# uzh-rpg/ess

Hardware: AMD Instinct MI355X
Metric: UDA train-step throughput (voxel grids/s = N*B*T/step_time) (higher is better)
Workload: dtype f16 forward / bf16 backward

## Files before the change

### ess_amd/csrc/conv_wgrad.hip

```cpp
#include "conv_wgrad_common.h"
#include <stdlib.h>

namespace {


__device__ __forceinline__ float load_virtual(const WgradArgs& a, int n, int c, int gy, int gx) {
  const bool first = c < a.C0;
  const int mode = first ? a.mode0 : a.mode1;
  const int sh = mode != ESS_SRC_DIRECT ? 1 : 0;
  const int Hp = a.Hin >> sh, Wp = a.Win >> sh;
  const float* sp = first ? a.src0 : a.src1;
  const int cc = first ? c : c - a.C0, Cs = first ? a.C0 : a.C1;
  const bool ok = gy >= 0 && gy < a.Hin && gx >= 0 && gx < a.Win && !(mode == ESS_SRC_ZERO_UP2 && ((gy | gx) & 1));
  const int cy = min(max(gy, 0), a.Hin - 1) >> sh, cx = min(max(gx, 0), a.Win - 1) >> sh;
  const float t = sp[(((size_t)n * Cs + cc) * Hp + cy) * Wp + cx];
  return ok ? t : 0.f;
}

__device__ __forceinline__ void load8_virtual(const WgradArgs& a, int n, int c, int gy, int gx, bool valid, float (&f)[8]) {
  const bool first = c < a.C0;
  const int mode = first ? a.mode0 : a.mode1;
  const float* sp = first ? a.src0 : a.src1;
  const int cc = first ? c : c - a.C0, Cs = first ? a.C0 : a.C1;
  const bool rowok = valid && gy >= 0 && gy < a.Hin;
// ... 686 lines not shown
  if (a.ws_b && tid < Cout) a.ws_b[(size_t)blockIdx.x * Cout + tid] = (redb[0][tid] + redb[1][tid]) + (redb[2][tid] + redb[3][tid]);
}

struct TapMap { int mapped; signed char m[12]; };
template <int E, int NT, int THREADS>
__global__ __launch_bounds__(THREADS) void wgrad_reduce_kernel(const float* ws, const float* ws_b, float* dw, float* db, int nsplit, int T,
                                                           int CC, int Cout, int nblk_w, int accumulate, const TapMap tm) {
  constexpr int G = THREADS / E, PITCH = E * NT + 1, U = NT == 1 ? 8 : 4;
  __shared__ float part[G * PITCH];
  int blk = blockIdx.x, t0 = blockIdx.y * NT, nt = min(NT, T - t0);
  if (blk >= nblk_w) {
    if (blockIdx.y) return;
    blk -= nblk_w; ws = ws_b; dw = db; T = 1; CC = Cout; nt = 1;
  }
  const bool mapped = tm.mapped && T == 9;
  const int el = threadIdx.x % E, g = threadIdx.x / E;
  const int e = blk * E + el;
  float acc[NT];
#pragma unroll
  for (int u = 0; u < NT; ++u) acc[u] = 0.f;
  if (e < CC) {
    int k = g;
    for (; k + (U - 1) * G < nsplit; k += U * G) {
      float v[U][NT];
#pragma unroll
      for (int j = 0; j < U; ++j) {
        const float* src = ws + ((size_t)(k + j * G) * T + t0) * CC + e;
#pragma unroll
        for (int u = 0; u < NT; ++u) v[j][u] = u < nt ? src[(size_t)u * CC] : 0.f;
      }
#pragma unroll
      for (int u = 0; u < NT; ++u) {
        float t = 0.f;
#pragma unroll
        for (int j = 0; j < U; j += 2) t += v[j][u] + v[j + 1][u];
        acc[u] += t;
      }
    }
    for (; k < nsplit; k += G) {
      const float* src = ws + ((size_t)k * T + t0) * CC + e;
#pragma unroll
      for (int u = 0; u < NT; ++u)
        if (u < nt) acc[u] += src[(size_t)u * CC];
    }
  }
#pragma unroll
  for (int u = 0; u < NT; ++u) part[g * PITCH + el * NT + u] = acc[u];
  __syncthreads();
  for (int idx = threadIdx.x; idx < E * NT; idx += THREADS) {
    const int l = idx / NT, u = idx - l * NT;
    if (u < nt && blk * E + l < CC) {
      float t = 0.f;
#pragma unroll
      for (int w = 0; w < G; ++w) t += part[w * PITCH + idx];
      const int td = mapped ? tm.m[t0 + u] : t0 + u;
      if (td < 0) continue;
      float* dst = dw + (size_t)(blk * E + l) * T + td;
      *dst = accumulate ? *dst + t : t;
    }
  }
}

enum WRoute {
  W_F32_TILE,
  W_TAPS7,
  W_BF16_K3,
  W_BF16_K3_FAST,
  W_BF16_K1,
  W_C8_K3,
  W_C8_K1,
  W_SMALL1X1,
  W_SMALL1X1_MFMA,
  W_SMALL1X1_C8X
};
inline bool tile128(WRoute r) { return r == W_BF16_K3 || r == W_BF16_K3_FAST || r == W_BF16_K1 || r == W_C8_K3 || r == W_C8_K1; }

struct WPlan {
  EssConvDesc d;
  WRoute route;
  bool phases;
  WgradBArgs args;
  unsigned grid;
  int lds_bytes;
  size_t ws_bytes;
};

inline bool k3s1p1(const EssConvDesc* d) { return d->ksize == 3 && d->stride == 1 && d->pad == 1; }

inline bool s2_phases(const EssConvDesc* d) {
  return d->fmt0 == ESS_FMT_BF16_C8 && d->fmt_out == ESS_FMT_BF16_C8 && d->ksize == 3 && d->stride == 2 && d->pad == 1 && d->C1 == 0 &&
         d->mode0 == ESS_SRC_DIRECT && d->H_in == 2 * d->H_out && d->W_in == 2 * d->W_out;
}
inline EssConvDesc s2_phase_desc(const EssConvDesc* d) {
  EssConvDesc p = *d;
  p.stride = 1; p.H_in = d->H_out; p.W_in = d->W_out; p.mode1 = ESS_SRC_DIRECT;
  return p;
}
inline TapMap s2_phase_taps(int p, int q) {
  TapMap tm{};
  tm.mapped = 1;
  for (int t = 0; t < 9; ++t) {
    const int kyp = t / 3, kxp = t % 3;
    const int ky = p == 0 ? (kyp == 1 ? 1 : -1) : (kyp == 0 ? 0 : kyp == 1 ? 2 : -1);
    const int kx = q == 0 ? (kxp == 1 ? 1 : -1) : (kxp == 0 ? 0 : kxp == 1 ? 2 : -1);
    tm.m[t] = (signed char)((ky < 0 || kx < 0) ? -1 : ky * 3 + kx);
  }
  return tm;
}

int wvalidate(const EssConvDesc* d) {
  ESS_CHECK_ARG(d != nullptr, "wgrad: null descriptor");
  ESS_CHECK_ARG(d->epilogue == ESS_EPI_LINEAR && d->out_split == 0, "wgrad: only plain convolutions have a weight gradient here");
  ESS_CHECK_ARG(d->mode0 >= ESS_SRC_DIRECT && d->mode0 <= ESS_SRC_ZERO_UP2 && d->mode1 >= ESS_SRC_DIRECT && d->mode1 <= ESS_SRC_ZERO_UP2,
                "wgrad: source modes DIRECT / NEAREST_UP2 / ZERO_UP2 only (the space-to-depth form exists for the frozen encoder's forward)");
  const int cin = d->C0 + d->C1;
  const bool taps = cin == 1 && d->ksize == 7;
  ESS_CHECK_ARG(taps || d->ksize == 1 || d->ksize == 3, "wgrad: k=%d with C_in=%d unsupported", d->ksize, cin);
  ESS_CHECK_ARG(d->stride == 1 || d->stride == 2, "wgrad: stride %d unsupported", d->stride);
  const bool xc8 = d->fmt0 == ESS_FMT_BF16_C8, dc8 = d->fmt_out == ESS_FMT_BF16_C8;
  ESS_CHECK_ARG(d->compute == ESS_COMPUTE_FP32 || d->compute == ESS_COMPUTE_BF16 || d->compute == ESS_COMPUTE_BF16X3, "wgrad: bad compute type");
  if (xc8 || dc8) {
    ESS_CHECK_ARG(d->compute == ESS_COMPUTE_BF16, "wgrad: BF16_C8 tensors need bf16 compute");
    ESS_CHECK_ARG(d->C1 == 0 || d->fmt1 == d->fmt0, "wgrad: both sources of a concat must use the same format");
    ESS_CHECK_ARG(d->C1 == 0 || (d->C0 % 8) == 0, "wgrad: the first BF16_C8 source of a concat must have a multiple of 8 channels");
    if (xc8 && dc8)
      ESS_CHECK_ARG(k3s1p1(d) || (d->ksize == 1 && d->pad == 0 && d->mode0 == ESS_SRC_DIRECT && d->C1 == 0) || s2_phases(d),
                    "wgrad(BF16_C8): 3x3 / stride 1 / pad 1, 3x3 / stride 2 / pad 1 on even extents (one direct source) and 1x1 / pad 0 convolutions only");
    else if (xc8)
      ESS_CHECK_ARG(d->ksize == 1 && d->stride == 1 && d->pad == 0 && d->C1 == 0 && d->mode0 == ESS_SRC_DIRECT && d->C_out <= 32 && cin <= 32,
                    "wgrad(BF16_C8 X, fp32 dY): the 1x1 head only (C_in, C_out <= 32)");
    else
      ESS_CHECK_ARG(taps, "wgrad(fp32 X, BF16_C8 dY): the 7x7 single-channel stem only");
  }
  return ESS_OK;
}

WRoute wroute(const EssConvDesc* d) {
  const int cin = d->C0 + d->C1, KS = d->ksize;
  const bool xc8 = d->fmt0 == ESS_FMT_BF16_C8, dc8 = d->fmt_out == ESS_FMT_BF16_C8;
  if (xc8 && dc8) return KS == 3 ? W_C8_K3 : W_C8_K1;
  if (xc8) return W_SMALL1X1_C8X;
  const bool k1s1p0 = KS == 1 && d->stride == 1 && d->pad == 0;
  if (k1s1p0 && d->C1 == 0 && d->mode0 == ESS_SRC_DIRECT && d->C_out <= 16 && cin <= 64)
    return cin <= 32 && ((d->H_out * d->W_out) % 64) == 0 ? W_SMALL1X1_MFMA : W_SMALL1X1;
  const bool rows8 = (d->W_in % 8) == 0 && (d->W_out % 8) == 0 && d->mode0 != ESS_SRC_ZERO_UP2 && d->mode1 != ESS_SRC_ZERO_UP2;
  if (d->compute == ESS_COMPUTE_BF16 && k3s1p1(d)) return rows8 ? W_BF16_K3_FAST : W_BF16_K3;
  if (d->compute == ESS_COMPUTE_BF16 && k1s1p0 && rows8) return W_BF16_K1;
  if (cin == 1 && KS == 7) return W_TAPS7;
  return W_F32_TILE;
}

WPlan wplan(const EssConvDesc* desc) {
  WPlan w{};
  w.d = *desc;
  if (desc->compute == ESS_COMPUTE_BF16X3) {
    w.args.split = k3s1p1(desc);
    w.d.compute = w.args.split ? ESS_COMPUTE_BF16 : ESS_COMPUTE_FP32;
  }
  w.phases = s2_phases(&w.d);
  if (w.phases) w.d = s2_phase_desc(&w.d);
  const EssConvDesc* d = &w.d;
  w.route = wroute(d);
  WgradArgs& a = w.args.w;
  a.N = d->N; a.Hin = d->H_in; a.Win = d->W_in; a.C0 = d->C0; a.C1 = d->C1; a.mode0 = d->mode0; a.mode1 = d->mode1;
  a.Cout = d->C_out; a.Hout = d->H_out; a.Wout = d->W_out;
  a.pad = (w.route == W_BF16_K1 || w.route == W_C8_K1) ? 1 : d->pad;
  a.dy_c8 = d->fmt_out == ESS_FMT_BF16_C8;
  a.ps = w.phases;
  const int cin = d->C0 + d->C1, KS = d->ksize, S = d->stride;
  const bool wide = tile128(w.route);
  const int npx = wide ? 128 : 64;
  double best = 1e300;
  for (int twl = 5; twl >= (wide ? 4 : 3); --twl) {
    const int tw = 1 << twl, th = npx >> twl;
    const double c = (double)ceil_div(d->W_out, tw) * tw * ceil_div(d->H_out, th) * th + 1e-3 * (5 - twl);
    if (c < best) { best = c; a.twl = twl; }
  }
  if (w.route == W_C8_K3) a.twl = 4;
  const int tw = 1 << a.twl, th = npx >> a.twl;
  a.tiles_x = ceil_div(d->W_out, tw); a.tiles_y = ceil_div(d->H_out, th);
  a.ntiles = d->N * a.tiles_x * a.tiles_y;
  a.IH = (th - 1) * S + KS; a.IW = (tw - 1) * S + KS;
  a.plx = (a.IH * a.IW) | 1;
  a.ci_tiles = w.route == W_TAPS7 ? 1 : ceil_div(cin, 64);
  a.npairs = ceil_div(d->C_out, 64) * a.ci_tiles;
  const size_t slab_floats = (size_t)KS * KS * d->C_out * cin + d->C_out;
  int ns = wide ? ceil_div(256, a.npairs) : ceil_div(2048, a.npairs);
  if (ns > a.ntiles) ns = a.ntiles;
  const size_t cap = ((size_t)64 << 20) / (slab_floats * 4);
  if ((size_t)ns > cap) ns = (int)(cap ? cap : 1);
  if (ns < 1) ns = 1;
  if (w.route == W_SMALL1X1 || w.route == W_SMALL1X1_C8X) {
    const int chunks = d->N * ceil_div(d->H_out * d->W_out, 128);
    ns = chunks < 1024 ? chunks : 1024;
  } else if (w.route == W_SMALL1X1_MFMA) {
    const int groups = d->N * (d->H_out * d->W_out / 64);
    ns = groups < 4 * 512 ? ceil_div(groups, 4) : 512;
  }
  a.nsplit = ns;
  w.grid = (unsigned)(a.npairs * ns);
  w.ws_bytes = (size_t)ns * slab_floats * 4;
  w.lds_bytes = (64 * 65 + (w.route == W_TAPS7 ? a.IH * a.IW : 64 * a.plx)) * 4;
  if (wide) {
    w.args.rv = tw / 8 + 2;
    w.args.pyv = (th * tw / 8) | 1;
    w.args.pxv = ((th + 2) * w.args.rv) | 1;
    w.lds_bytes = 64 * (w.args.pyv + w.args.pxv) * 16 * (w.route == W_BF16_K3 ? 1 : 2);
  }
  return w;
}

struct WgradSet { const void* x0; const void* x1; const void* dy; };

WgradBArgs wfill(const WPlan& w, const WgradSet& s, void* workspace, bool bias, int ph) {
  WgradBArgs b = w.args;
  WgradArgs& a = b.w;
  a.src0 = (const float*)s.x0; a.src1 = a.C1 ? (const float*)s.x1 : nullptr; a.dy = (const float*)s.dy;
  a.ws = (float*)workspace;
  a.ws_b = bias ? a.ws + (size_t)a.nsplit * w.d.ksize * w.d.ksize * a.Cout * (a.C0 + a.C1) : nullptr;
  a.pp = ph >> 1; a.pq = ph & 1;
  return b;
}

template <typename K, typename... A>
int wgo(K kernel, dim3 grid, int lds_bytes, hipStream_t st, const A&... args) {
  const int rc = wgrad_raise_lds(kernel, lds_bytes);
  if (rc) return rc;
  hipLaunchKernelGGL(kernel, grid, dim3(256), lds_bytes, st, args...);
  return ESS_OK;
}

int wlaunch(const WPlan& w, WRoute route, const WgradBArgs& b, hipStream_t st) {
  const EssConvDesc& d = w.d;
  const dim3 grid(w.grid);
  const int px = d.H_out * d.W_out, nsplit = b.w.nsplit;
  int rc = ESS_OK;
  switch (route) {
    case W_F32_TILE: {
      const auto kernel = d.ksize == 3 ? (d.stride == 1 ? wgrad_f32_kernel<3, 1> : wgrad_f32_kernel<3, 2>)
                                       : (d.stride == 1 ? wgrad_f32_kernel<1, 1> : wgrad_f32_kernel<1, 2>);
      rc = wgo(kernel, grid, w.lds_bytes, st, b.w);
      break;
    }
    case W_TAPS7: rc = wgo(wgrad_taps_kernel<7, 2>, grid, w.lds_bytes, st, b.w); break;
    case W_BF16_K3: rc = wgo(wgrad_bf16_k3s1_kernel, grid, w.lds_bytes, st, b); break;
    case W_BF16_K3_FAST: rc = wgo(wgrad_bf16_k3s1_fast_kernel<9>, grid, w.lds_bytes, st, b); break;
    case W_BF16_K1: rc = wgo(wgrad_bf16_k3s1_fast_kernel<1>, grid, w.lds_bytes, st, b); break;
    case W_C8_K3: rc = wgrad_c8_k3_launch(b, grid, st); break;
    case W_C8_K1: rc = wgrad_c8_k1_launch(b, d.stride, w.lds_bytes, grid, st); break;
    case W_SMALL1X1: rc = wgo(wgrad_small1x1_kernel, dim3(nsplit), 0, st, b.w, ceil_div(px, 128), d.N * ceil_div(px, 128)); break;
    case W_SMALL1X1_MFMA: rc = wgo(wgrad_small1x1_mfma_kernel, dim3(nsplit), 0, st, b.w, px / 64, d.N * (px / 64)); break;
    case W_SMALL1X1_C8X: rc = wgrad_small1x1_c8_launch(b.w, nsplit, st); break;
  }
  return rc ? rc : ess_launch_status("conv2d_wgrad");
}

int wreduce(const WPlan& w, const WgradArgs& a, float* dw, float* db, int accumulate, const TapMap& tm, hipStream_t st) {
  const int T = w.d.ksize * w.d.ksize, CC = w.d.C_out * (w.d.C0 + w.d.C1);
  const int nblk_w = ceil_div(CC, 64), nblk_b = a.ws_b ? ceil_div(w.d.C_out, 64) : 0;
  if (T == 9 && CC >= 32768)
    hipLaunchKernelGGL((wgrad_reduce_kernel<64, 9, 256>), dim3((unsigned)(nblk_w + nblk_b)), dim3(256), 0, st, a.ws, a.ws_b, dw, db, a.nsplit, T,
                       CC, w.d.C_out, nblk_w, accumulate, tm);
  else
    hipLaunchKernelGGL((wgrad_reduce_kernel<64, 1, 1024>), dim3((unsigned)(nblk_w + nblk_b), (unsigned)T), dim3(1024), 0, st, a.ws, a.ws_b, dw, db,
                       a.nsplit, T, CC, w.d.C_out, nblk_w, accumulate, tm);
  return ess_launch_status("conv2d_wgrad_reduce");
}

bool env_on(const char* name) {
  const char* e = getenv(name);
  return !(e && e[0] == '0');
}

bool split_via_c8(const EssConvDesc* d) {
  static const bool on = env_on("ESS_X3_WGRAD_C8");
  return on && d->compute == ESS_COMPUTE_BF16X3 && k3s1p1(d) && (d->C1 == 0 || (d->C0 % 8) == 0) && d->mode0 != ESS_SRC_ZERO_UP2 &&
         d->mode1 != ESS_SRC_ZERO_UP2 && (d->C1 == 0 || d->mode1 == ESS_SRC_DIRECT);
}
EssConvDesc c8_desc(const EssConvDesc* d) {
  EssConvDesc c = *d;
  c.compute = ESS_COMPUTE_BF16;
  c.fmt0 = c.fmt1 = c.fmt_out = ESS_FMT_BF16_C8;
  return c;
}
struct SplitCopy { int C, H, W; size_t bytes; };
struct SplitLayout { size_t slabs, total; SplitCopy t[3]; };
SplitLayout split_layout(const EssConvDesc* d) {
  const EssConvDesc dc = c8_desc(d);
  const int s0 = d->mode0 != ESS_SRC_DIRECT ? 1 : 0, s1 = d->mode1 != ESS_SRC_DIRECT ? 1 : 0;
  SplitLayout s{(wplan(&dc).ws_bytes + 255) & ~(size_t)255, 0,
                {{d->C0, d->H_in >> s0, d->W_in >> s0, 0}, {d->C1, d->H_in >> s1, d->W_in >> s1, 0}, {d->C_out, d->H_out, d->W_out, 0}}};
  s.total = s.slabs;
  for (SplitCopy& t : s.t) {
    t.bytes = (((size_t)d->N * ((t.C + 7) / 8) * t.H * t.W * 16) + 255) & ~(size_t)255;
    s.total += 2 * t.bytes;
  }
  return s;
}

int wgrad_split_via_c8(const EssConvDesc* d, const WgradSet& s, float* dw, float* db, int accumulate, void* workspace, size_t workspace_bytes,
                       hipStream_t st);

int wgrad_run(const EssConvDesc* d, int n_sets, const WgradSet* sets, int bias_mask, float* dw, float* db, int accumulate, void* workspace,
              size_t workspace_bytes, hipStream_t st) {
  int rc = wvalidate(d);
  if (rc) return rc;
  ESS_CHECK_ARG(dw && workspace, "wgrad: null pointer");
  uintptr_t bits = 0;
  for (int q = 0; q < n_sets; ++q) {
    ESS_CHECK_ARG(sets[q].x0 && sets[q].dy, "wgrad: null pointer");
    ESS_CHECK_ARG(d->C1 == 0 || sets[q].x1, "wgrad: second source missing");
    bits |= (uintptr_t)sets[q].x0 | (uintptr_t)sets[q].dy | (d->C1 ? (uintptr_t)sets[q].x1 : 0);
  }
  if (split_via_c8(d)) {
    for (int q = 0; q < n_sets; ++q)
      if ((rc = wgrad_split_via_c8(d, sets[q], dw, ((bias_mask >> q) & 1) ? db : nullptr, q ? 1 : accumulate, workspace, workspace_bytes, st))) return rc;
    return ESS_OK;
  }
  const WPlan w = wplan(d);
  ESS_CHECK_ARG(workspace_bytes >= w.ws_bytes, "wgrad: workspace too small");
  ESS_CHECK_ARG(w.lds_bytes <= 160 * 1024, "wgrad: LDS tile %d B too large", w.lds_bytes);
  if (w.d.fmt0 == ESS_FMT_BF16_C8 || w.d.fmt_out == ESS_FMT_BF16_C8)
    ESS_CHECK_ARG((bits & 15) == 0, "wgrad: BF16_C8 tensors must be 16-byte aligned");
  if (w.route == W_TAPS7) {
    ESS_CHECK_ARG(w.d.stride == 2, "wgrad: 7x7 stem variant is stride 2 only");
    ESS_CHECK_ARG(!db, "wgrad: the stem variant has no bias gradient");
  }
  const bool one_launch = n_sets > 1 && w.route == W_C8_K3 && !w.phases;
  for (int q = 0; q < (one_launch ? 1 : n_sets); ++q) {
    const bool misaligned = (((uintptr_t)sets[q].x0 | (uintptr_t)sets[q].dy) & 15) != 0;
    const WRoute route = (w.route == W_SMALL1X1_MFMA && misaligned) ? W_SMALL1X1 : w.route;
    for (int ph = 0; ph < (w.phases ? 4 : 1); ++ph) {
      const bool bias = db && ph == 0 && (one_launch || ((bias_mask >> q) & 1));
      WgradBArgs b = wfill(w, sets[q], workspace, bias, ph);
      if (one_launch) {
        b.npass = n_sets; b.bias_mask = bias_mask;
        for (int i = 0; i < n_sets; ++i) { b.p_dy[i] = sets[i].dy; b.p_x0[i] = sets[i].x0; b.p_x1[i] = d->C1 ? sets[i].x1 : nullptr; }
      }
      if ((rc = wlaunch(w, route, b, st))) return rc;
      if ((rc = wreduce(w, b.w, dw, db, (q || accumulate) ? 1 : 0, w.phases ? s2_phase_taps(ph >> 1, ph & 1) : TapMap{}, st))) return rc;
    }
  }
  return ESS_OK;
}

int wgrad_split_via_c8(const EssConvDesc* d, const WgradSet& s, float* dw, float* db, int accumulate, void* workspace,
                              size_t workspace_bytes, hipStream_t st) {
  int rc;
// ... 46 lines not shown
```

### ess_amd/csrc/conv_wgrad_c8.hip

```cpp
#include "conv_wgrad_common.h"
#include <stdlib.h>
#include <type_traits>

namespace {

struct Quad { u32x4w v[4]; };

__device__ __forceinline__ void quad_transpose(const Quad& q, uint2 (&out)[8]) {
#pragma unroll
  for (int d = 0; d < 4; ++d) {
    out[2 * d].x = __builtin_amdgcn_perm(q.v[1][d], q.v[0][d], 0x05040100u);
    out[2 * d].y = __builtin_amdgcn_perm(q.v[3][d], q.v[2][d], 0x05040100u);
    out[2 * d + 1].x = __builtin_amdgcn_perm(q.v[1][d], q.v[0][d], 0x07060302u);
    out[2 * d + 1].y = __builtin_amdgcn_perm(q.v[3][d], q.v[2][d], 0x07060302u);
  }
}

template <int OFF>
__device__ __forceinline__ void lds_read128(u32x4w& d, unsigned addr) {
  asm volatile("ds_read_b128 %0, %1 offset:%2" : "=v"(d) : "v"(addr), "n"(OFF));
}

template <int TAPS, int TWL>
__global__ __launch_bounds__(256) void wgrad_c8_kernel(const WgradBArgs b, int sx_abl) {
// ... 150 lines not shown
    auto mma = [&](const Frag& f) {
      if (abl & 1) return;
      const bf16x8w af = __builtin_bit_cast(bf16x8w, f.a);
      if (want_b) {
#pragma unroll
        for (int j = 0; j < 8; ++j) bsum += (float)af[j];
      }
      if constexpr (TAPS == 1) {
        acc[0] = __builtin_amdgcn_mfma_f32_32x32x16_bf16(af, __builtin_bit_cast(bf16x8w, f.v[1][1]), acc[0], 0, 0, 0);
      } else {
#pragma unroll
        for (int ky = 0; ky < 3; ++ky) {
          acc[ky * 3 + 0] = __builtin_amdgcn_mfma_f32_32x32x16_bf16(af, __builtin_bit_cast(bf16x8w, shift_left1(f.v[ky][0], f.v[ky][1])),
                                                                    acc[ky * 3 + 0], 0, 0, 0);
          acc[ky * 3 + 1] = __builtin_amdgcn_mfma_f32_32x32x16_bf16(af, __builtin_bit_cast(bf16x8w, f.v[ky][1]), acc[ky * 3 + 1], 0, 0, 0);
          acc[ky * 3 + 2] = __builtin_amdgcn_mfma_f32_32x32x16_bf16(af, __builtin_bit_cast(bf16x8w, shift_right1(f.v[ky][1], f.v[ky][2])),
                                                                    acc[ky * 3 + 2], 0, 0, 0);
        }
      }
    };
    Frag f0, f1;
    ESS_RD(f0, 0)
    ESS_RD(f1, 1) ESS_WT(f0, NR) mma(f0);
    if (more) issue(tile + nsplit);
    ESS_RD(f0, 2) ESS_WT(f1, NR) mma(f1);
    ESS_RD(f1, 3) ESS_WT(f0, NR) mma(f0);
    ESS_RD(f0, 4) ESS_WT(f1, NR) mma(f1);
    if (more) commit_d(st ^ 1);
    ESS_RD(f1, 5) ESS_WT(f0, NR) mma(f0);
    if (more) commit_x(0, st ^ 1);
    ESS_RD(f0, 6) ESS_WT(f1, NR) mma(f1);
    if (more) commit_x(1, st ^ 1);
    ESS_RD(f1, 7) ESS_WT(f0, NR) mma(f0);
    if (more) commit_x(2, st ^ 1);
    ESS_WT(f1, 0) mma(f1);
#undef ESS_RD
#undef ESS_WT
#undef ESS_ROFF
    __syncthreads();
  }
  const int ci = cit * 64 + ib * 32 + p;
  if (abl & 8) return;
#pragma unroll
  for (int t = 0; t < TAPS; ++t)
#pragma unroll
    for (int r = 0; r < 16; ++r) {
      const int co = cot * 64 + cb * 32 + (r & 3) + 8 * (r >> 2) + 4 * half;
      if (co < a.Cout && ci < Cin) a.ws[(((size_t)split * TAPS + t) * a.Cout + co) * Cin + ci] = acc[t][r];
    }
  if (want_b) {
    bsum += __shfl_xor(bsum, 32, 64);
    const int co = cot * 64 + cb * 32 + p;
    if (half == 0 && co < a.Cout) a.ws_b[(size_t)split * a.Cout + co] = bsum;
  }
}

template <int OFF>
__device__ __forceinline__ void lds_read_tr(uint2& d, unsigned addr) {
  asm volatile("ds_read_b64_tr_b16 %0, %1 offset:%2" : "=v"(d) : "v"(addr), "n"(OFF));
}
template <int I, int N, class F>
__device__ __forceinline__ void static_for(F&& f) {
  if constexpr (I < N) {
    f(std::integral_constant<int, I>{});
    static_for<I + 1, N>(f);
  }
}
#define ESS_LDS_PTR(off_) ((__attribute__((address_space(3))) void*)(size_t)(off_))

struct DmaGeom {
  static constexpr int TWL = 4, TW = 16, TH = 8, RW = TW + 2, IH = TH + 2, XPX = IH * RW;
  static constexpr int XP = (XPX + 63) / 64, XTAIL = XPX - (XP - 1) * 64;
  static constexpr int DPL = 2 * 1024 + 64, XPL = XPX * 16;
  static_assert(XPL % 256 == 64, "X plane pitch");
  static constexpr int XREG = 8 * DPL, STAGE = 8 * (DPL + XPL);
};

#ifdef ESS_WG_TRACE
__device__ unsigned long long g_wg_trace[1024 * 8 * 40];
#define ESS_TR(i_) do { if (lane == 0 && blockIdx.x < 1024) g_wg_trace[(blockIdx.x * 8 + wave) * 40 + (i_)] = __builtin_readcyclecounter(); } while (0)
#else
#define ESS_TR(i_) do { } while (0)
#endif
template <int NST>
__global__ __launch_bounds__(512) void wgrad_c8_ws_kernel(const WgradBArgs b) {
  using G = DmaGeom;
  constexpr int PER_WAVE = 2 * (2 + G::XP);
  constexpr int AHEAD = 2;
  static_assert(NST == AHEAD + 2, "stages: tile k - 1 (last two units), k, k + 1 (landing), k + 2 (being issued)");
  extern __shared__ __attribute__((aligned(16))) unsigned char smem_dma[];
  const WgradArgs& a = b.w;
  const int tid = threadIdx.x, lane = tid & 63, wave = __builtin_amdgcn_readfirstlane(tid >> 6), half = lane >> 5, p = lane & 31;
  const bool loader = wave >= 4;
  const int w4 = wave & 3;
  const int logical = xcd_remap(blockIdx.x, gridDim.x);
  const int pair = logical % a.npairs, split = logical / a.npairs, nsplit = a.nsplit;
  const int cot = pair / a.ci_tiles, cit = pair - cot * a.ci_tiles;
  const int Cin = a.C0 + a.C1;
  const unsigned lds0 = (unsigned)(size_t)smem_dma;
  const int ntt = b.npass > 1 ? b.npass * a.ntiles : a.ntiles;
  int ntl = 0;
  if (split < ntt) ntl = (ntt - 1 - split) / nsplit + 1;

  ESS_TR(0);
  if (loader) {
    const int sh0 = a.mode0 != ESS_SRC_DIRECT ? 1 : 0, sh1 = a.mode1 != ESS_SRC_DIRECT ? 1 : 0;
    const bool z0 = a.mode0 == ESS_SRC_ZERO_UP2, z1 = a.mode1 == ESS_SRC_ZERO_UP2;
    const int nbo = (a.Cout + 7) >> 3, nb0 = (a.C0 + 7) >> 3, nb1 = (a.C1 + 7) >> 3;
    const unsigned HWo16 = (unsigned)a.Hout * a.Wout * 16u;
    const int W0 = (a.Win << a.ps) >> sh0, W1 = a.Win >> sh1;
    const unsigned HW0_16 = (unsigned)((a.Hin << a.ps) >> sh0) * W0 * 16u, HW1_16 = (unsigned)(a.Hin >> sh1) * W1 * 16u;
    int d_r[2], d_c[2], x_r[G::XP], x_c[G::XP];
#pragma unroll
    for (int q = 0; q < 2; ++q) { const int pi = q * 64 + lane; d_r[q] = pi >> G::TWL; d_c[q] = pi & (G::TW - 1); }
#pragma unroll
    for (int q = 0; q < G::XP; ++q) { const int pi = q * 64 + lane; x_r[q] = pi / G::RW; x_c[q] = pi % G::RW; }
    unsigned dpl_off[2], xpl_off[2];
    bool xpl_first[2];
#pragma unroll
    for (int j = 0; j < 2; ++j) {
      const int pl = 2 * w4 + j;
      const int ob = cot * 8 + pl;
      dpl_off[j] = ob < nbo ? (unsigned)ob * HWo16 : OOBW;
      const int c0 = (cit * 8 + pl) * 8;
      const bool first = c0 < a.C0 || a.C1 == 0;
      const int bi = (first ? c0 : c0 - a.C0) >> 3;
      xpl_first[j] = first;
      xpl_off[j] = (c0 < Cin && bi < (first ? nb0 : nb1)) ? (unsigned)bi * (first ? HW0_16 : HW1_16) : OOBW;
    }
    const int tpi = a.tiles_x * a.tiles_y;
    auto issue = [&](int tile, int st) {
      const char* p_dy = (const char*)a.dy;
      const char* p_x0 = (const char*)a.src0;
      const char* p_x1 = (const char*)a.src1;
      if (b.npass > 1) {
        const int pass = tile / a.ntiles;
        tile -= pass * a.ntiles;
        p_dy = (const char*)(pass == 0 ? b.p_dy[0] : pass == 1 ? b.p_dy[1] : b.p_dy[2]);
        p_x0 = (const char*)(pass == 0 ? b.p_x0[0] : pass == 1 ? b.p_x0[1] : b.p_x0[2]);
        p_x1 = (const char*)(pass == 0 ? b.p_x1[0] : pass == 1 ? b.p_x1[1] : b.p_x1[2]);
      }
      if (!a.C1) p_x1 = p_x0;
      const int n = tile / tpi;
      const int tr = tile - n * tpi;
      const int ty = tr / a.tiles_x, tx = tr - ty * a.tiles_x;
      const int y0 = ty * G::TH, x0 = tx * G::TW;
      const __amdgpu_buffer_rsrc_t r_dy =
          __builtin_amdgcn_make_buffer_rsrc((void*)(p_dy + (size_t)n * nbo * HWo16), 0, (int)(nbo * HWo16), 0x00020000);
      const __amdgpu_buffer_rsrc_t r_x0 =
          __builtin_amdgcn_make_buffer_rsrc((void*)(p_x0 + (size_t)n * nb0 * HW0_16), 0, (int)(nb0 * HW0_16), 0x00020000);
      const __amdgpu_buffer_rsrc_t r_x1 = __builtin_amdgcn_make_buffer_rsrc(
          (void*)(p_x1 + (size_t)n * (a.C1 ? nb1 * HW1_16 : 0u)), 0, (int)(a.C1 ? nb1 * HW1_16 : 0u), 0x00020000);
      const unsigned sbase = lds0 + (unsigned)st * G::STAGE;
      unsigned vd[2], vx0[G::XP], vx1[G::XP];
#pragma unroll
      for (int q = 0; q < 2; ++q) {
        const int y = y0 + d_r[q], x = x0 + d_c[q];
        const bool in = (y < a.Hout) & (x < a.Wout);
        vd[q] = in ? (unsigned)(y * a.Wout + x) * 16u : OOBW;
      }
#pragma unroll
      for (int q = 0; q < G::XP; ++q) {
        const int gy = y0 - 1 + x_r[q], gx = x0 - 1 + x_c[q];
        const bool in = ((unsigned)gy < (unsigned)a.Hin) & ((unsigned)gx < (unsigned)a.Win);
        const bool odd = (gy | gx) & 1;
        vx0[q] = (in & !(z0 & odd)) ? (unsigned)((((gy << a.ps) + a.pp) >> sh0) * W0 + (((gx << a.ps) + a.pq) >> sh0)) * 16u : OOBW;
        vx1[q] = (in & !(z1 & odd)) ? (unsigned)((gy >> sh1) * W1 + (gx >> sh1)) * 16u : OOBW;
      }
#pragma unroll
      for (int j = 0; j < 2; ++j) {
        const int pl = 2 * w4 + j;
#pragma unroll
        for (int q = 0; q < 2; ++q) {
          const unsigned vo = (dpl_off[j] | vd[q]) & OOBW ? OOBW : dpl_off[j] + vd[q];
          __builtin_amdgcn_raw_ptr_buffer_load_lds(r_dy, ESS_LDS_PTR(sbase + pl * G::DPL + q * 1024), 16, (int)vo, 0, 0, 0);
        }
#pragma unroll
        for (int q = 0; q < G::XP; ++q) {
          const unsigned vq = xpl_first[j] ? vx0[q] : vx1[q];
          const unsigned vo = (xpl_off[j] | vq) & OOBW ? OOBW : xpl_off[j] + vq;
          if (q < G::XP - 1 || lane < G::XTAIL) {
            if (xpl_first[j])
              __builtin_amdgcn_raw_ptr_buffer_load_lds(r_x0, ESS_LDS_PTR(sbase + G::XREG + pl * G::XPL + q * 1024), 16, (int)vo, 0, 0, 0);
            else
              __builtin_amdgcn_raw_ptr_buffer_load_lds(r_x1, ESS_LDS_PTR(sbase + G::XREG + pl * G::XPL + q * 1024), 16, (int)vo, 0, 0, 0);
          }
        }
      }
    };
    ESS_TR(1);
    for (int k = 0; k < AHEAD && k < ntl; ++k) issue(split + k * nsplit, k);
    ESS_TR(2);
    for (int k = 0; k < ntl; ++k) {
      if (k < 30) ESS_TR(3 + k);
      if (k + 1 < ntl) asm volatile("s_waitcnt vmcnt(%0)" ::"n"(PER_WAVE) : "memory");
      else asm volatile("s_waitcnt vmcnt(0)" ::: "memory");
      __builtin_amdgcn_s_barrier();
      if (k + AHEAD < ntl) issue(split + (k + AHEAD) * nsplit, (k + AHEAD) % NST);
    }
    ESS_TR(37);
    return;
  }

  const int cb = w4 >> 1, ib = w4 & 1;
  f32x16 acc[9];
#pragma unroll
  for (int t = 0; t < 9; ++t)
#pragma unroll
    for (int r = 0; r < 16; ++r) acc[t][r] = 0.f;
  float bsum = 0.f;
  const bool want_b0 = a.ws_b && cit == 0 && ib == 0;
  bool want_b = want_b0;
  const int g = lane >> 4, i16 = lane & 15;
  const unsigned pix_off = (unsigned)((8 * (g >> 1) + (i16 >> 2)) * 16 + (i16 & 1) * 8);
  const unsigned pl_sel = (unsigned)(2 * (g & 1) + ((i16 & 3) >> 1));
  const unsigned a_lane = (unsigned)(cb * 4 + pl_sel) * G::DPL + pix_off;
  const unsigned x_lane = G::XREG + (unsigned)(ib * 4 + pl_sel) * G::XPL + pix_off;
  struct FA { uint2 lo, hi; };
  struct FB { uint2 lo[3], hi[3]; };
  FA fa[2];
  FB fb[3];
  unsigned a_addr = lds0 + a_lane, x_addr = lds0 + x_lane, a_next = 0, x_next = 0;
  auto rd = [&](auto uc, unsigned aad, unsigned xad) {
    constexpr int U = decltype(uc)::value, KS = U / 3, KY = U % 3;
    if constexpr (KY == 0) {
      lds_read_tr<KS * 256>(fa[KS & 1].lo, aad);
      lds_read_tr<KS * 256 + 64>(fa[KS & 1].hi, aad);
    }
    constexpr int XO = (KS + KY) * G::RW * 16;
    lds_read_tr<XO + 0>(fb[U % 3].lo[0], xad);
    lds_read_tr<XO + 64>(fb[U % 3].hi[0], xad);
    lds_read_tr<XO + 16>(fb[U % 3].lo[1], xad);
    lds_read_tr<XO + 80>(fb[U % 3].hi[1], xad);
    lds_read_tr<XO + 32>(fb[U % 3].lo[2], xad);
    lds_read_tr<XO + 96>(fb[U % 3].hi[2], xad);
  };
  auto unit = [&](auto uc, auto nextc) {
    constexpr int U = decltype(uc)::value, KS = U / 3, KY = U % 3;
    constexpr bool NEXT = decltype(nextc)::value;
    if constexpr (U + 2 < 24) rd(std::integral_constant<int, U + 2>{}, a_addr, x_addr);
    else if constexpr (NEXT) rd(std::integral_constant<int, U + 2 - 24>{}, a_next, x_next);
    constexpr int N1 = (U + 1 < 24 || NEXT) ? 6 + ((U + 1) % 3 == 0 ? 2 : 0) : 0, N2 = (U + 2 < 24 || NEXT) ? 6 + ((U + 2) % 3 == 0 ? 2 : 0) : 0;
    constexpr int LEFT = N1 + N2;
    FA& A_ = fa[KS & 1];
    FB& B_ = fb[U % 3];
    if constexpr (KY == 0)
      asm volatile("s_waitcnt lgkmcnt(%8)"
                   : "+v"(A_.lo), "+v"(A_.hi), "+v"(B_.lo[0]), "+v"(B_.hi[0]), "+v"(B_.lo[1]), "+v"(B_.hi[1]), "+v"(B_.lo[2]), "+v"(B_.hi[2])
                   : "n"(LEFT));
    else
      asm volatile("s_waitcnt lgkmcnt(%6)"
                   : "+v"(B_.lo[0]), "+v"(B_.hi[0]), "+v"(B_.lo[1]), "+v"(B_.hi[1]), "+v"(B_.lo[2]), "+v"(B_.hi[2])
                   : "n"(LEFT));
    const u32x4w av = {A_.lo.x, A_.lo.y, A_.hi.x, A_.hi.y};
    const bf16x8w af = __builtin_bit_cast(bf16x8w, av);
    if constexpr (KY == 0) {
      if (want_b) {
#pragma unroll
        for (int jj = 0; jj < 8; ++jj) bsum += (float)af[jj];
      }
    }
#pragma unroll
    for (int kx = 0; kx < 3; ++kx) {
      const u32x4w xv = {B_.lo[kx].x, B_.lo[kx].y, B_.hi[kx].x, B_.hi[kx].y};
      acc[KY * 3 + kx] = __builtin_amdgcn_mfma_f32_32x32x16_bf16(af, __builtin_bit_cast(bf16x8w, xv), acc[KY * 3 + kx], 0, 0, 0);
    }
  };
  using Yes = std::true_type;
  using No = std::false_type;
  ESS_TR(1);
  if (ntl > 0) {
    __builtin_amdgcn_s_barrier();
    rd(std::integral_constant<int, 0>{}, a_addr, x_addr);
    rd(std::integral_constant<int, 1>{}, a_addr, x_addr);
  }
  for (int k = 0; k + 1 < ntl; ++k) {
    if (k < 30) ESS_TR(3 + k);
    if (b.npass > 1) want_b = want_b0 && ((b.bias_mask >> ((split + k * nsplit) / a.ntiles)) & 1);
    const unsigned nst = (unsigned)((k + 1) % NST) * G::STAGE;
    a_next = lds0 + nst + a_lane;
    x_next = lds0 + nst + x_lane;
    static_for<0, 22>([&](auto uc) { unit(uc, No{}); });
    __builtin_amdgcn_s_barrier();
    unit(std::integral_constant<int, 22>{}, Yes{});
    unit(std::integral_constant<int, 23>{}, Yes{});
    a_addr = a_next;
    x_addr = x_next;
  }
  if (ntl > 0) {
    if (ntl - 1 < 30) ESS_TR(3 + ntl - 1);
    if (b.npass > 1) want_b = want_b0 && ((b.bias_mask >> ((split + (ntl - 1) * nsplit) / a.ntiles)) & 1);
    static_for<0, 24>([&](auto uc) { unit(uc, No{}); });
  }
  ESS_TR(34);
  const int ci = cit * 64 + ib * 32 + p, co0 = cot * 64 + cb * 32 + 4 * half;
  float* wsp = a.ws + ((size_t)split * 9 * a.Cout + co0) * Cin + ci;
  const int tap_stride = a.Cout * Cin;
  if (ci < Cin) {
#pragma unroll
    for (int r = 0; r < 16; ++r) {
      const int dco = (r & 3) + 8 * (r >> 2);
      if (co0 + dco < a.Cout) {
        float* q = wsp + dco * Cin;
#pragma unroll
        for (int t = 0; t < 9; ++t) q[t * tap_stride] = acc[t][r];
      }
    }
  }
  if (want_b) {
    bsum += __shfl_xor(bsum, 32, 64);
    const int co = cot * 64 + cb * 32 + p;
    if (half == 0 && co < a.Cout) a.ws_b[(size_t)split * a.Cout + co] = bsum;
  }
  ESS_TR(37);
}

__global__ __launch_bounds__(256) void wgrad_small1x1_c8_kernel(const WgradArgs a, int chunks_per_img, int total_chunks) {
  constexpr int P = 128, PP = P + 1;
  __shared__ float dy_s[32 * PP];
  __shared__ float x_s[32 * PP];
  float* red = dy_s;
  const int tid = threadIdx.x, lane = tid & 63, wave = tid >> 6, half = lane >> 5, p = lane & 31;
  const int Cin = a.C0, Cout = a.Cout, nbi = (Cin + 7) >> 3;
  const size_t HW = (size_t)a.Hout * a.Wout;
  f32x16 acc;
#pragma unroll
  for (int r = 0; r < 16; ++r) acc[r] = 0.f;
  float bsum = 0.f;
  for (int i = tid; i < 32 * PP; i += 256) { dy_s[i] = 0.f; x_s[i] = 0.f; }
  for (int chunk = blockIdx.x; chunk < total_chunks; chunk += gridDim.x) {
    const int n = chunk / chunks_per_img;
    const size_t px0 = (size_t)(chunk - n * chunks_per_img) * P;
    __syncthreads();
    for (int i = tid; i < nbi * P; i += 256) {
      const int blk = i / P, j = i - blk * P;
      const size_t px = px0 + j;
      const u32x4w v = ((const u32x4w*)a.src0)[((size_t)n * nbi + blk) * HW + (px < HW ? px : HW - 1)];
      const unsigned m = px < HW ? 0xffffffffu : 0u;
#pragma unroll
      for (int q = 0; q < 4; ++q) {
        x_s[(blk * 8 + 2 * q) * PP + j] = __builtin_bit_cast(float, (v[q] << 16) & m);
        x_s[(blk * 8 + 2 * q + 1) * PP + j] = __builtin_bit_cast(float, v[q] & 0xffff0000u & m);
      }
    }
    for (int i = tid; i < Cout * P; i += 256) {
      const int r = i / P, j = i - r * P;
      const size_t px = px0 + j;
      const float t = a.dy[((size_t)n * Cout + r) * HW + (px < HW ? px : HW - 1)];
      dy_s[r * PP + j] = px < HW ? t : 0.f;
    }
    __syncthreads();
    const float* dp = dy_s + p * PP + wave * 32 + half;
    const float* xp = x_s + p * PP + wave * 32 + half;
#pragma unroll 8
    for (int kk = 0; kk < 16; ++kk) {
      const float d1 = dp[2 * kk], x1 = xp[2 * kk];
      bsum += d1;
      acc = __builtin_amdgcn_mfma_f32_32x32x2f32(d1, x1, acc, 0, 0, 0);
    }
  }
  __syncthreads();
  float* redb = x_s;
#pragma unroll
  for (int r = 0; r < 16; ++r) red[wave * 1024 + r * 64 + lane] = acc[r];
  bsum += __shfl_xor(bsum, 32, 64);
  if (half == 0) redb[wave * 32 + p] = bsum;
  __syncthreads();
  for (int i = tid; i < 16 * 64; i += 256) {
    const int r = i >> 6, l = i & 63;
    const int co = (r & 3) + 8 * (r >> 2) + 4 * (l >> 5), ci = l & 31;
    if (co < Cout && ci < Cin)
      a.ws[(size_t)blockIdx.x * Cout * Cin + co * Cin + ci] = (red[i] + red[1024 + i]) + (red[2048 + i] + red[3072 + i]);
  }
  if (a.ws_b && tid < Cout) a.ws_b[(size_t)blockIdx.x * Cout + tid] = (redb[tid] + redb[32 + tid]) + (redb[64 + tid] + redb[96 + tid]);
}

}

int wgrad_c8_k3_launch(const WgradBArgs& b, dim3 grid, hipStream_t st) {
  if (b.w.twl != 4) { ess_set_error("wgrad(BF16_C8, 3x3): stride 1, 16-wide pixel tiles"); return ESS_EINVAL; }
  constexpr int NST = 4, lds = NST * DmaGeom::STAGE;
  static_assert(lds <= 160 * 1024, "LDS stages of the weight-gradient kernel");
  const int rc = wgrad_raise_lds(wgrad_c8_ws_kernel<NST>, lds);
  if (rc) return rc;
  hipLaunchKernelGGL((wgrad_c8_ws_kernel<NST>), grid, dim3(512), lds, st, b);
  return ess_launch_status("conv2d_wgrad(BF16_C8, LDS-DMA, loader waves)");
}

int wgrad_c8_k1_launch(const WgradBArgs& b, int sx, int lds_bytes, dim3 grid, hipStream_t st) {
  if (b.w.twl != 4 && b.w.twl != 5) { ess_set_error("wgrad(BF16_C8): pixel tiles are 16 or 32 wide"); return ESS_EINVAL; }
  const auto kernel = b.w.twl == 5 ? wgrad_c8_kernel<1, 5> : wgrad_c8_kernel<1, 4>;
  const int rc = wgrad_raise_lds(kernel, lds_bytes);
  if (rc) return rc;
  hipLaunchKernelGGL(kernel, grid, dim3(256), lds_bytes, st, b, sx);
  return ess_launch_status("conv2d_wgrad(BF16_C8)");
}

int wgrad_small1x1_c8_launch(const WgradArgs& a, int nsplit, hipStream_t st) {
  const int per_img = ceil_div(a.Hout * a.Wout, 128);
  hipLaunchKernelGGL(wgrad_small1x1_c8_kernel, dim3(nsplit), dim3(256), 0, st, a, per_img, a.N * per_img);
  return ess_launch_status("conv2d_wgrad(1x1 head, BF16_C8)");
}

#ifdef ESS_WG_TRACE
extern "C" int ess_debug_wgrad_trace(unsigned long long* host_out, size_t n) {
  return (int)hipMemcpyFromSymbol(host_out, HIP_SYMBOL(g_wg_trace), n * sizeof(unsigned long long));
}
#endif
```

### ess_amd/csrc/conv_wgrad_common.h

```cpp
#pragma once
#include "common.h"

struct WgradArgs {
  const float* src0;
  const float* src1;
  const float* dy;
  float* ws;
  float* ws_b;
  int N, Hin, Win, C0, C1, mode0, mode1, Cout, Hout, Wout, pad;
  int twl;
  int tiles_x, tiles_y, ntiles;
  int IH, IW, plx;
  int ci_tiles, npairs, nsplit;
  int dy_c8;
  int ps, pp, pq;
};

constexpr unsigned OOBW = 0x80000000u;
typedef __bf16 bf16x8w __attribute__((ext_vector_type(8)));
typedef unsigned int u32x4w __attribute__((ext_vector_type(4)));


__device__ __forceinline__ u32x4w cvt8(const float (&v)[8]) {
  bf16x8w b;
#pragma unroll
  for (int j = 0; j < 8; ++j) b[j] = (__bf16)v[j];
  return __builtin_bit_cast(u32x4w, b);
}
__device__ __forceinline__ u32x4w cvt8_lo(const float (&v)[8]) {
  bf16x8w b;
#pragma unroll
  for (int j = 0; j < 8; ++j) b[j] = (__bf16)(v[j] - (float)(__bf16)v[j]);
  return __builtin_bit_cast(u32x4w, b);
}
__device__ __forceinline__ u32x4w shift_left1(u32x4w lo, u32x4w hi) {
  u32x4w r;
  r[0] = __builtin_amdgcn_alignbyte(hi[0], lo[3], 2);
  r[1] = __builtin_amdgcn_alignbyte(hi[1], hi[0], 2);
  r[2] = __builtin_amdgcn_alignbyte(hi[2], hi[1], 2);
  r[3] = __builtin_amdgcn_alignbyte(hi[3], hi[2], 2);
  return r;
}
__device__ __forceinline__ u32x4w shift_right1(u32x4w lo, u32x4w hi) {
  u32x4w r;
  r[0] = __builtin_amdgcn_alignbyte(lo[1], lo[0], 2);
  r[1] = __builtin_amdgcn_alignbyte(lo[2], lo[1], 2);
  r[2] = __builtin_amdgcn_alignbyte(lo[3], lo[2], 2);
  r[3] = __builtin_amdgcn_alignbyte(hi[0], lo[3], 2);
  return r;
}


struct WgradBArgs {
  WgradArgs w;
  int pyv, pxv, rv;
  int split;
  int npass;
  int bias_mask;
  const void* p_dy[3];
  const void* p_x0[3];
  const void* p_x1[3];
};

template <typename K>
int wgrad_raise_lds(K kernel, int bytes) {
  if (bytes > 64 * 1024) {
    hipError_t e = hipFuncSetAttribute((const void*)kernel, hipFuncAttributeMaxDynamicSharedMemorySize, bytes);
    if (e != hipSuccess) {
      ess_set_error("hipFuncSetAttribute(%d B LDS): %s", bytes, hipGetErrorString(e));
      return ESS_ELAUNCH;
    }
  }
  return ESS_OK;
}

int wgrad_c8_k3_launch(const WgradBArgs& b, dim3 grid, hipStream_t st);
int wgrad_c8_k1_launch(const WgradBArgs& b, int sx, int lds_bytes, dim3 grid, hipStream_t st);
int wgrad_small1x1_c8_launch(const WgradArgs& a, int nsplit, hipStream_t st);
int ess_split_bf16_c8_internal(const float* x, void* hi, void* lo, int N, int C, int H, int W, hipStream_t st);
```

Baseline: 1683.

## Add narrow wgrad variant for 3x3 C8 convs with at most 32 output channels

For the LDS-DMA 3x3 BF16_C8 weight-gradient kernel, layers with at most 32 output channels get a narrow template. It loads only one dy plane pair per wave and runs half the MFMA units per tile. The two channel-block halves instead cover different pixel halves and write separate workspace slabs, which doubles the slab count that the reduce kernel sums. The goal is to avoid wasted loads and MFMA work on padded output channels, at the cost of a larger workspace, a halved split cap and a longer reduction.

```diff
diff --git a/ess_amd/csrc/conv_wgrad.hip b/ess_amd/csrc/conv_wgrad.hip
--- a/ess_amd/csrc/conv_wgrad.hip
+++ b/ess_amd/csrc/conv_wgrad.hip
@@ -792,8 +792,15 @@
   WgradBArgs args;
   unsigned grid;
   int lds_bytes;
+  bool narrow;
+  int nslabs;
   size_t ws_bytes;
 };
+
+inline bool wgrad_narrow_on() {
+  static const bool on = [] { const char* e = getenv("ESS_WGRAD_NARROW"); return !(e && e[0] == '0'); }();
+  return on;
+}
 
 inline bool k3s1p1(const EssConvDesc* d) { return d->ksize == 3 && d->stride == 1 && d->pad == 1; }
 
@@ -897,7 +904,8 @@
   const size_t slab_floats = (size_t)KS * KS * d->C_out * cin + d->C_out;
   int ns = wide ? ceil_div(256, a.npairs) : ceil_div(2048, a.npairs);
   if (ns > a.ntiles) ns = a.ntiles;
-  const size_t cap = ((size_t)64 << 20) / (slab_floats * 4);
+  w.narrow = w.route == W_C8_K3 && d->C_out <= 32 && a.ntiles > 1 && wgrad_narrow_on();
+  const size_t cap = ((size_t)64 << 20) / (slab_floats * 4) / (w.narrow ? 2 : 1);
   if ((size_t)ns > cap) ns = (int)(cap ? cap : 1);
   if (ns < 1) ns = 1;
   if (w.route == W_SMALL1X1 || w.route == W_SMALL1X1_C8X) {
@@ -909,7 +917,8 @@
   }
   a.nsplit = ns;
   w.grid = (unsigned)(a.npairs * ns);
-  w.ws_bytes = (size_t)ns * slab_floats * 4;
+  w.nslabs = w.narrow ? 2 * ns : ns;
+  w.ws_bytes = (size_t)w.nslabs * slab_floats * 4;
   w.lds_bytes = (64 * 65 + (w.route == W_TAPS7 ? a.IH * a.IW : 64 * a.plx)) * 4;
   if (wide) {
     w.args.rv = tw / 8 + 2;
@@ -927,7 +936,7 @@
   WgradArgs& a = b.w;
   a.src0 = (const float*)s.x0; a.src1 = a.C1 ? (const float*)s.x1 : nullptr; a.dy = (const float*)s.dy;
   a.ws = (float*)workspace;
-  a.ws_b = bias ? a.ws + (size_t)a.nsplit * w.d.ksize * w.d.ksize * a.Cout * (a.C0 + a.C1) : nullptr;
+  a.ws_b = bias ? a.ws + (size_t)w.nslabs * w.d.ksize * w.d.ksize * a.Cout * (a.C0 + a.C1) : nullptr;
   a.pp = ph >> 1; a.pq = ph & 1;
   return b;
 }
@@ -956,7 +965,7 @@
     case W_BF16_K3: rc = wgo(wgrad_bf16_k3s1_kernel, grid, w.lds_bytes, st, b); break;
     case W_BF16_K3_FAST: rc = wgo(wgrad_bf16_k3s1_fast_kernel<9>, grid, w.lds_bytes, st, b); break;
     case W_BF16_K1: rc = wgo(wgrad_bf16_k3s1_fast_kernel<1>, grid, w.lds_bytes, st, b); break;
-    case W_C8_K3: rc = wgrad_c8_k3_launch(b, grid, st); break;
+    case W_C8_K3: rc = wgrad_c8_k3_launch(b, w.narrow, grid, st); break;
     case W_C8_K1: rc = wgrad_c8_k1_launch(b, d.stride, w.lds_bytes, grid, st); break;
     case W_SMALL1X1: rc = wgo(wgrad_small1x1_kernel, dim3(nsplit), 0, st, b.w, ceil_div(px, 128), d.N * ceil_div(px, 128)); break;
     case W_SMALL1X1_MFMA: rc = wgo(wgrad_small1x1_mfma_kernel, dim3(nsplit), 0, st, b.w, px / 64, d.N * (px / 64)); break;
@@ -969,11 +978,11 @@
   const int T = w.d.ksize * w.d.ksize, CC = w.d.C_out * (w.d.C0 + w.d.C1);
   const int nblk_w = ceil_div(CC, 64), nblk_b = a.ws_b ? ceil_div(w.d.C_out, 64) : 0;
   if (T == 9 && CC >= 32768)
-    hipLaunchKernelGGL((wgrad_reduce_kernel<64, 9, 256>), dim3((unsigned)(nblk_w + nblk_b)), dim3(256), 0, st, a.ws, a.ws_b, dw, db, a.nsplit, T,
+    hipLaunchKernelGGL((wgrad_reduce_kernel<64, 9, 256>), dim3((unsigned)(nblk_w + nblk_b)), dim3(256), 0, st, a.ws, a.ws_b, dw, db, w.nslabs, T,
                        CC, w.d.C_out, nblk_w, accumulate, tm);
   else
     hipLaunchKernelGGL((wgrad_reduce_kernel<64, 1, 1024>), dim3((unsigned)(nblk_w + nblk_b), (unsigned)T), dim3(1024), 0, st, a.ws, a.ws_b, dw, db,
-                       a.nsplit, T, CC, w.d.C_out, nblk_w, accumulate, tm);
+                       w.nslabs, T, CC, w.d.C_out, nblk_w, accumulate, tm);
   return ess_launch_status("conv2d_wgrad_reduce");
 }
 
diff --git a/ess_amd/csrc/conv_wgrad_c8.hip b/ess_amd/csrc/conv_wgrad_c8.hip
--- a/ess_amd/csrc/conv_wgrad_c8.hip
+++ b/ess_amd/csrc/conv_wgrad_c8.hip
@@ -256,10 +256,12 @@
 #else
 #define ESS_TR(i_) do { } while (0)
 #endif
-template <int NST>
+template <int NST, bool NARROW = false>
 __global__ __launch_bounds__(512) void wgrad_c8_ws_kernel(const WgradBArgs b) {
   using G = DmaGeom;
-  constexpr int PER_WAVE = 2 * (2 + G::XP);
+  constexpr int NDJ = NARROW ? 1 : 2;
+  constexpr int PER_WAVE = 2 * NDJ + 2 * G::XP;
+  constexpr int NU = NARROW ? 12 : 24;
   constexpr int AHEAD = 2;
   static_assert(NST == AHEAD + 2, "stages: tile k - 1 (last two units), k, k + 1 (landing), k + 2 (being issued)");
   extern __shared__ __attribute__((aligned(16))) unsigned char smem_dma[];
@@ -294,7 +296,7 @@
 #pragma unroll
     for (int j = 0; j < 2; ++j) {
       const int pl = 2 * w4 + j;
-      const int ob = cot * 8 + pl;
+      const int ob = cot * 8 + (NARROW ? w4 : pl);
       dpl_off[j] = ob < nbo ? (unsigned)ob * HWo16 : OOBW;
       const int c0 = (cit * 8 + pl) * 8;
       const bool first = c0 < a.C0 || a.C1 == 0;
@@ -344,10 +346,13 @@
 #pragma unroll
       for (int j = 0; j < 2; ++j) {
         const int pl = 2 * w4 + j;
-#pragma unroll
-        for (int q = 0; q < 2; ++q) {
-          const unsigned vo = (dpl_off[j] | vd[q]) & OOBW ? OOBW : dpl_off[j] + vd[q];
-          __builtin_amdgcn_raw_ptr_buffer_load_lds(r_dy, ESS_LDS_PTR(sbase + pl * G::DPL + q * 1024), 16, (int)vo, 0, 0, 0);
+        if (j < NDJ) {
+          const int dpl = NARROW ? w4 : pl;
+#pragma unroll
+          for (int q = 0; q < 2; ++q) {
+            const unsigned vo = (dpl_off[j] | vd[q]) & OOBW ? OOBW : dpl_off[j] + vd[q];
+            __builtin_amdgcn_raw_ptr_buffer_load_lds(r_dy, ESS_LDS_PTR(sbase + dpl * G::DPL + q * 1024), 16, (int)vo, 0, 0, 0);
+          }
         }
 #pragma unroll
         for (int q = 0; q < G::XP; ++q) {
@@ -388,8 +393,8 @@
   const int g = lane >> 4, i16 = lane & 15;
   const unsigned pix_off = (unsigned)((8 * (g >> 1) + (i16 >> 2)) * 16 + (i16 & 1) * 8);
   const unsigned pl_sel = (unsigned)(2 * (g & 1) + ((i16 & 3) >> 1));
-  const unsigned a_lane = (unsigned)(cb * 4 + pl_sel) * G::DPL + pix_off;
-  const unsigned x_lane = G::XREG + (unsigned)(ib * 4 + pl_sel) * G::XPL + pix_off;
+  const unsigned a_lane = NARROW ? pl_sel * G::DPL + pix_off + (unsigned)cb * (4 * G::TW * 16) : (unsigned)(cb * 4 + pl_sel) * G::DPL + pix_off;
+  const unsigned x_lane = G::XREG + (unsigned)(ib * 4 + pl_sel) * G::XPL + pix_off + (NARROW ? (unsigned)cb * (4 * G::RW * 16) : 0u);
   struct FA { uint2 lo, hi; };
   struct FB { uint2 lo[3], hi[3]; };
   FA fa[2];
@@ -412,9 +417,9 @@
   auto unit = [&](auto uc, auto nextc) {
     constexpr int U = decltype(uc)::value, KS = U / 3, KY = U % 3;
     constexpr bool NEXT = decltype(nextc)::value;
-    if constexpr (U + 2 < 24) rd(std::integral_constant<int, U + 2>{}, a_addr, x_addr);
-    else if constexpr (NEXT) rd(std::integral_constant<int, U + 2 - 24>{}, a_next, x_next);
-    constexpr int N1 = (U + 1 < 24 || NEXT) ? 6 + ((U + 1) % 3 == 0 ? 2 : 0) : 0, N2 = (U + 2 < 24 || NEXT) ? 6 + ((U + 2) % 3 == 0 ? 2 : 0) : 0;
+    if constexpr (U + 2 < NU) rd(std::integral_constant<int, U + 2>{}, a_addr, x_addr);
+    else if constexpr (NEXT) rd(std::integral_constant<int, U + 2 - NU>{}, a_next, x_next);
+    constexpr int N1 = (U + 1 < NU || NEXT) ? 6 + ((U + 1) % 3 == 0 ? 2 : 0) : 0, N2 = (U + 2 < NU || NEXT) ? 6 + ((U + 2) % 3 == 0 ? 2 : 0) : 0;
     constexpr int LEFT = N1 + N2;
     FA& A_ = fa[KS & 1];
     FB& B_ = fb[U % 3];
@@ -454,21 +459,22 @@
     const unsigned nst = (unsigned)((k + 1) % NST) * G::STAGE;
     a_next = lds0 + nst + a_lane;
     x_next = lds0 + nst + x_lane;
-    static_for<0, 22>([&](auto uc) { unit(uc, No{}); });
+    static_for<0, NU - 2>([&](auto uc) { unit(uc, No{}); });
     __builtin_amdgcn_s_barrier();
-    unit(std::integral_constant<int, 22>{}, Yes{});
-    unit(std::integral_constant<int, 23>{}, Yes{});
+    unit(std::integral_constant<int, NU - 2>{}, Yes{});
+    unit(std::integral_constant<int, NU - 1>{}, Yes{});
     a_addr = a_next;
     x_addr = x_next;
   }
   if (ntl > 0) {
     if (ntl - 1 < 30) ESS_TR(3 + ntl - 1);
     if (b.npass > 1) want_b = want_b0 && ((b.bias_mask >> ((split + (ntl - 1) * nsplit) / a.ntiles)) & 1);
-    static_for<0, 24>([&](auto uc) { unit(uc, No{}); });
+    static_for<0, NU>([&](auto uc) { unit(uc, No{}); });
   }
   ESS_TR(34);
-  const int ci = cit * 64 + ib * 32 + p, co0 = cot * 64 + cb * 32 + 4 * half;
-  float* wsp = a.ws + ((size_t)split * 9 * a.Cout + co0) * Cin + ci;
+  const int slab = NARROW ? 2 * split + cb : split;
+  const int ci = cit * 64 + ib * 32 + p, co0 = cot * 64 + (NARROW ? 0 : cb * 32) + 4 * half;
+  float* wsp = a.ws + ((size_t)slab * 9 * a.Cout + co0) * Cin + ci;
   const int tap_stride = a.Cout * Cin;
   if (ci < Cin) {
 #pragma unroll
@@ -483,8 +489,8 @@
   }
   if (want_b) {
     bsum += __shfl_xor(bsum, 32, 64);
-    const int co = cot * 64 + cb * 32 + p;
-    if (half == 0 && co < a.Cout) a.ws_b[(size_t)split * a.Cout + co] = bsum;
+    const int co = cot * 64 + (NARROW ? 0 : cb * 32) + p;
+    if (half == 0 && co < a.Cout) a.ws_b[(size_t)slab * a.Cout + co] = bsum;
   }
   ESS_TR(37);
 }
@@ -551,10 +557,17 @@
 
 }
 
-int wgrad_c8_k3_launch(const WgradBArgs& b, dim3 grid, hipStream_t st) {
+int wgrad_c8_k3_launch(const WgradBArgs& b, bool narrow, dim3 grid, hipStream_t st) {
   if (b.w.twl != 4) { ess_set_error("wgrad(BF16_C8, 3x3): stride 1, 16-wide pixel tiles"); return ESS_EINVAL; }
   constexpr int NST = 4, lds = NST * DmaGeom::STAGE;
   static_assert(lds <= 160 * 1024, "LDS stages of the weight-gradient kernel");
+  if (narrow) {
+    if (b.w.Cout > 32) { ess_set_error("wgrad(BF16_C8, 3x3): the narrow form takes at most 32 output channels"); return ESS_EINVAL; }
+    const int rc = wgrad_raise_lds(wgrad_c8_ws_kernel<NST, true>, lds);
+    if (rc) return rc;
+    hipLaunchKernelGGL((wgrad_c8_ws_kernel<NST, true>), grid, dim3(512), lds, st, b);
+    return ess_launch_status("conv2d_wgrad(BF16_C8, LDS-DMA, loader waves, narrow)");
+  }
   const int rc = wgrad_raise_lds(wgrad_c8_ws_kernel<NST>, lds);
   if (rc) return rc;
   hipLaunchKernelGGL((wgrad_c8_ws_kernel<NST>), grid, dim3(512), lds, st, b);
diff --git a/ess_amd/csrc/conv_wgrad_common.h b/ess_amd/csrc/conv_wgrad_common.h
--- a/ess_amd/csrc/conv_wgrad_common.h
+++ b/ess_amd/csrc/conv_wgrad_common.h
@@ -74,7 +74,7 @@
   return ESS_OK;
 }
 
-int wgrad_c8_k3_launch(const WgradBArgs& b, dim3 grid, hipStream_t st);
+int wgrad_c8_k3_launch(const WgradBArgs& b, bool narrow, dim3 grid, hipStream_t st);
 int wgrad_c8_k1_launch(const WgradBArgs& b, int sx, int lds_bytes, dim3 grid, hipStream_t st);
 int wgrad_small1x1_c8_launch(const WgradArgs& a, int nsplit, hipStream_t st);
 int ess_split_bf16_c8_internal(const float* x, void* hi, void* lo, int N, int C, int H, int W, hipStream_t st);
```

Result: no change. 1690, median of 6 (+0.4%).
